# simonmeister/UnFlow

Hardware: AMD Instinct MI355X
Metric: image-pairs/s (fwd+bwd) FlowNetC 384x512 (higher is better)
Workload: dtype f32; 1 GPU; FlowNetC unsupervised step: bidirectional fwd + census/2nd-order loss pyramid + bwd + L2/Adam, 4 pairs/GPU, 384x512, 441-ch correlation (BASELINE configs[1]); global_batch=4, height=384, width=512, parallelism=dp1, hipgraph=True

## Files before the change

### include/unflow_hip.h

```cpp
#ifndef UNFLOW_HIP_H_
#define UNFLOW_HIP_H_

#include <stddef.h>

#ifdef __cplusplus
extern "C" {
#endif

typedef void* unflow_stream_t;
typedef struct unflow_planes unflow_planes;

#define UNFLOW_OK 0
#define UNFLOW_ERR_NULL (-1)
#define UNFLOW_ERR_EMPTY_OUTPUT (-2)
#define UNFLOW_ERR_EVEN_KERNEL (-3)
#define UNFLOW_ERR_NOT_DIVISIBLE (-4)
#define UNFLOW_ERR_SHAPE (-5)
#define UNFLOW_ERR_UNSUPPORTED (-7)
#define UNFLOW_ERR_LAUNCH (-8)
#define UNFLOW_ERR_WORKSPACE (-9)

const char* unflow_status_string(int status);
int unflow_version(void);

// ... 216 lines not shown

size_t unflow_conv_pl_workspace_bytes(int B, int H, int W, int Cin, int Cout, int k, int stride, int n_planes);

size_t unflow_flow_wgrad_batched_workspace_bytes(int n, const int* kind, const int* B, const int* H, const int* W, const int* Cin);
int unflow_flow_wgrad_batched(int n, const int* kind, const float* const* x, const int* ldx, const float* const* dz,
                              const int* lddz, float* const* dw, const int* B, const int* H, const int* W, const int* Cin,
                              void* workspace, size_t workspace_bytes, unflow_stream_t stream);

int unflow_debug_work_order(int mt, int nt, int ncls, int nsplit, int order, int xcd, int* out, int out_blocks);

int unflow_comm_available(void);
int unflow_comm_unique_id(void* id128);
int unflow_comm_init(const void* id128, int nranks, int rank, void** comm);
int unflow_comm_info(void* comm, int* nranks, int* rank);
int unflow_allreduce_sum_f32(float* buf, long n, void* comm, unflow_stream_t stream);
int unflow_comm_destroy(void* comm);

int unflow_debug_streamk_plan(int G, int mtp, int nt, int nchunk, int ncls, const int* ntaps, int ngroups, int* range_pos, int npos,
                              const int* pos, int* decoded);
int unflow_debug_streamk_timeouts(void);

int unflow_conv2d_fwd_pl(const float* x, int ldx, const unflow_planes* x_pl, const float* w, const unflow_planes* w_pl,
                         const float* bias, float* y, int ldy, const unflow_planes* y_pl, int B, int H, int W, int Cin,
                         int Cout, int k, int stride, int leaky, void* workspace, size_t workspace_bytes,
                         unflow_stream_t stream);
int unflow_conv2d_bwd_data_pl(const float* dz, int lddz, const unflow_planes* dz_pl, const float* w,
                              const unflow_planes* w_pl, float* dx, int lddx, const unflow_planes* dx_pl, int pl_lo,
                              int pl_hi, int B, int H, int W, int Cin, int Cout, int k, int stride, int accumulate,
                              const float* act_src, int ld_act, const unflow_planes* act_pl, int act_lo, int act_hi,
                              void* workspace, size_t workspace_bytes, unflow_stream_t stream);
int unflow_conv2d_bwd_filter_pl(const float* x, int ldx, const unflow_planes* x_pl, const float* dz, int lddz,
                                const unflow_planes* dz_pl, float* dw, int B, int H, int W, int Cin, int Cout, int k,
                                int stride, void* workspace, size_t workspace_bytes, unflow_stream_t stream);
int unflow_conv2d_transpose_fwd_pl(const float* x, int ldx, const unflow_planes* x_pl, const float* w,
                                   const unflow_planes* w_pl, const float* bias, float* y, int ldy,
                                   const unflow_planes* y_pl, int B, int H, int W, int Cin, int Cout, int leaky,
                                   void* workspace, size_t workspace_bytes, unflow_stream_t stream);
int unflow_conv2d_transpose_bwd_data_pl(const float* dz, int lddz, const unflow_planes* dz_pl, const float* w,
                                        const unflow_planes* w_pl, float* dx, int lddx, const unflow_planes* dx_pl,
                                        int pl_lo, int pl_hi, int B, int H, int W, int Cin, int Cout, int accumulate,
                                        const float* act_src, int ld_act, const unflow_planes* act_pl, int act_lo,
                                        int act_hi, void* workspace, size_t workspace_bytes, unflow_stream_t stream);
int unflow_conv2d_transpose_bwd_filter_pl(const float* x, int ldx, const unflow_planes* x_pl, const float* dz, int lddz,
                                          const unflow_planes* dz_pl, float* dw, int B, int H, int W, int Cin, int Cout,
                                          void* workspace, size_t workspace_bytes, unflow_stream_t stream);

int unflow_resize_bilinear_tf1(const float* in, float* out, int B, int H, int W, int C, int out_h, int out_w,
                               float scale, unflow_stream_t stream);

int unflow_supervised_flow_loss(const float* flow, int h, int w, const float* flow_gt, const float* mask_gt, float flow_scale,
                                float weight, float* loss_acc, float* d_flow, int accumulate, int B, int H, int W,
                                unflow_stream_t stream);

int unflow_stack_input_pair(const float* first4, const float* second4, const float* prev_flow2, float* out, int ld_out, int N,
                            int H, int W, int h, int w, float flow_scale, unflow_stream_t stream);
int unflow_stack_input_pair_bwd(const float* d_out, int ld_out, const float* first4, const float* second4,
                                const float* prev_flow2, float* d_prev_flow2, int N, int H, int W, int h, int w,
                                float flow_scale, unflow_stream_t stream);

int unflow_adam_step(float* p, const float* grad, float* m, float* v, long n, long n_regularized, float grad_scale,
                     float l2_scale, float lr_t, float beta1, float beta2, float eps, unflow_stream_t stream);

int unflow_adam_step_regloss(float* p, const float* grad, float* m, float* v, long n, long n_regularized,
                             float grad_scale, float l2_scale, float lr_t, float beta1, float beta2, float eps,
                             float* loss_acc, unflow_stream_t stream);

// ... 107 lines not shown
```

### unflow_amd/core/engine.py

```python
import math
import os
from collections import OrderedDict

import numpy as np
import torch

from .. import _lib
from .._lib import check, ptr, stream, cf, cl
from . import layers as L

FLOW_SCALE = 5.0
CHANNEL_MEAN = [104.920005, 110.1753, 114.785955]
LAYER_WEIGHTS = [12.7, 4.35, 3.9, 3.4, 1.1]
LAYER_PATCH_DISTANCES = [3, 2, 2, 1, 1]
LAYER_WEIGHTS_FULL_RES = [12.7, 5.5, 5.0, 4.35, 3.9, 3.4, 1.1]
LAYER_PATCH_DISTANCES_FULL_RES = [3, 3] + LAYER_PATCH_DISTANCES
L2_SCALE = 0.0004
LOSSES = ['occ', 'sym', 'fb', 'grad', 'ternary', 'photo', 'smooth_1st', 'smooth_2nd']

DEFAULT_PARAMS = dict(flownet='C', pyramid_loss=True, border_mask=True, ternary_weight=1.0, smooth_2nd_weight=3.0)


def pad4(c):
    return (c + 3) // 4 * 4


def round8(c):
    return (c + 7) // 8 * 8


def conv_math_mode():
    m = os.environ.get('UNFLOW_CONV_MATH', 'bf16x3')
    if m not in ('bf16x3', 'fp32', 'f16'):
        raise ValueError("UNFLOW_CONV_MATH must be bf16x3, fp32 or f16")
    return m


RGB4_FORM = True


class Layer:
    __slots__ = ('name', 'kind', 'k', 'cin', 'cout', 'stride', 'act', 'cin_p', 'cout_p', 'in_map', 'w', 'b', 'dw', 'db', 'mw', 'vw', 'mb', 'vb',
                 'wpl_d', 'wpl_t')

    def __init__(self, name, kind, k, cin, cout, stride, act, in_map=None, cin_p=None):
        self.name, self.kind, self.k, self.cin, self.cout, self.stride, self.act = name, kind, k, cin, cout, stride, act
        self.in_map = in_map or [(0, 0, cin)]
        if cin_p is None:
            cin_p = cin if (kind == 'deconv' and cin == 2) else pad4(max(lo + n for lo, _, n in self.in_map))
        self.cin_p = cin_p
        self.cout_p = cout if cout <= 2 else pad4(cout)
        self.wpl_d = self.wpl_t = None

    def wshape(self):
        if self.kind == 'conv':
            return (self.k, self.k, self.cin_p, self.cout_p)
        return (self.k, self.k, self.cout_p, self.cin_p)

    def tf_wshape(self):
        return (self.k, self.k, self.cin, self.cout) if self.kind == 'conv' else (self.k, self.k, self.cout, self.cin)

    def wplane_view(self):
        if self.kind == 'conv' and self.k == 7 and self.stride == 2 and self.cin_p == 4 and RGB4_FORM:
            return (7, 28, self.cout_p)
        return (self.k * self.k, self.wshape()[2], self.wshape()[3])

    def uses_planes(self):
        return self.cout > 4 and self.cin_p >= 4


def concat_layout(parts):
    off, d = 0, {}
    for nm, n in parts:
        off = pad4(off)
        d[nm] = (off, n)
        off += n
    return d, pad4(off)


class ActView(dict):

    def __init__(self, stage):
        super().__init__()
        self._stage = stage

# ... 393 lines not shown
            if e.wgrad_sync_each:
                main.wait_stream(side)

        flow_jobs = []
        n_flow = sum(1 for op, _, _, _ in self.bwd[lo:hi] if op.kind == 'layer' and op.l.cout <= 2) if e.batch_flow_wgrad else 0

        for k, (op, first, act_lo, act_hi) in enumerate(self.bwd[lo:hi], lo):
            if op.kind == 'corr':
                c3, g3, gout = self.pt(op.src), self.pt(op.src, True), self.pt(op.dst, True)
                C = op.src[2] - op.src[1]
                h8, w8 = e.H // 8, e.W // 8
                assert first
                pl = self._corr_planes(c3)
                if e.supervised:
                    p0, p1 = (None, None) if pl is None else (_lib.planes_of(pl[:, :B]), _lib.planes_of(pl[:, B:]))
                    check(_lib.lib().unflow_correlation_nhwc_bwd_pl(ptr(gout.t), gout.t.stride(2), ptr(c3.t[:B]), ptr(c3.t[B:]),
                                                                    c3.t.stride(2), p0, p1, 0, ptr(g3.t[:B]), ptr(g3.t[B:]),
                                                                    g3.t.stride(2), 0, B, C, h8, w8, 1, 20, 20, 1, 2, e.stream()),
                          "correlation_grad")
                else:
                    c3pl = _lib.planes_of(pl)
                    check(_lib.lib().unflow_correlation_nhwc_bwd_pl(ptr(gout.t), gout.t.stride(2), ptr(c3.t), ptr(c3.t),
                                                                    c3.t.stride(2), c3pl, c3pl, B, ptr(g3.t), ptr(None),
                                                                    g3.t.stride(2), 1, N, C, h8, w8, 1, 20, 20, 1, 2, e.stream()),
                          "correlation_grad")
                for r0, r1, clo, chi in self.bwd_post_act.get(k, ()):
                    self._leaky_bwd_rows(g3, c3, r0, r1, clo, chi)
                continue
            l = op.l
            x, dz = _rows(self.pt(op.src), op.n), _rows(self.pt(op.dst, True), op.n)
            if l.cout_p != l.cout:
                dz = L.PT(dz.t.as_strided(dz.t.shape[:3] + (l.cout_p,), dz.t.stride(), dz.t.storage_offset()), dz.pl, dz.scale)
            if e._bias_plan is None:
                e._bias_jobs.append((dz.t, l))
            xv = op.src[0] not in self.planes_only
            wg = (L.conv_bwd_filter, (x, dz, l.dw, l.stride, xv)) if l.kind == 'conv' else (L.deconv_bwd_filter, (x, dz, l.dw, xv))
            if n_flow and l.cout <= 2:
                flow_jobs.append((l.kind, x, dz, l.dw))
                wg = (L.flow_wgrad_batched, (flow_jobs,)) if len(flow_jobs) == n_flow else None
            if wg is None:
                pass
            elif side is None or (e.wgrad_inline_tiny and l.cout <= 2):
                wg[0](*wg[1])
            else:
                pending.append(wg)
                if len(pending) >= e.wgrad_group:
                    flush()
            sb = op.src[0]
            is_input = sb == 'x0' or (sb == self.bin and op.src[1] == 0 and op.src[2] == pad4(self.in_ch)
                                      and op.l.name.endswith('conv1'))
            if sb not in self.Gd or (is_input and not self.need_in_grad):
                continue
            dx = _rows(self.pt(op.src, True), op.n)
            accumulate = (not first) or sb.startswith('flow')
            if k in self.bwd_zero_rows:
                r0, r1 = self.bwd_zero_rows[k]
                gz = self.Gd[sb].t[r0:r1]
                check(_lib.lib().unflow_zero(ptr(gz), _lib.csz(gz.numel() * 4), e.stream()), "zero")
            act_src = _rows(self.pt(op.src), op.n) if act_hi > act_lo else None
            apl = sb in self.planes_only
            if l.kind == 'conv':
                L.conv_bwd_data(dz, l.w, l.wpl_d, dx, l.stride, accumulate, act_src, act_lo, act_hi, act_planes=apl)
            else:
                L.deconv_bwd_data(dz, l.w, l.wpl_t, dx, accumulate, act_src, act_lo, act_hi, act_planes=apl)
        if side is not None:
            flush()
        if before_join is not None:
            before_join()
        if side is not None:
# ... 996 lines not shown
```

### unflow_amd/core/layers.py

```python
import torch

from .. import _lib
from .._lib import check, ptr, stream, csz
from ..ops import workspace


def nhwc(t):
    assert t.dim() == 4 and t.dtype == torch.float32 and t.is_cuda, "NHWC float32 CUDA tensor expected"
    B, H, W, C = t.shape
    ld = t.stride(2)
    assert t.stride(3) == 1 and t.stride(1) == W * ld and t.stride(0) == H * W * ld, \
        "tensor must be a channel-slice view of a contiguous NHWC buffer"
    return ptr(t), ld, B, H, W, C


def out_hw(H, W, stride):
    return -(-H // stride), -(-W // stride)


_WS_SLOT = [1]


class ws_slot:

# ... 155 lines not shown
    k = w.shape[0]
    assert tuple(w.shape) == (k, k, Cin, Cout) and w.is_contiguous() and (Ho, Wo) == out_hw(H, W, stride)
    wsp, wsn = _ws_pl(x.t.device, B, H, W, Cin, Cout, k, stride, _npl(x, y))
    check(_lib.lib().unflow_conv2d_fwd_pl(xp, ldx, x.planes(), ptr(w), _lib.planes_of(w_pl), ptr(bias), yp, ldy,
                                          y.planes(), B, H, W, Cin, Cout, k, stride, int(bool(leaky)), wsp, wsn,
                                          stream()), "conv2d_fwd_pl")


def _act_args(act_src, act_planes):
    if act_src is None:
        return ptr(None), 0, None
    a = _pt(act_src)
    if act_planes:
        assert a.pl is not None
        return ptr(None), 0, a.planes()
    ap, lda = nhwc(a.t)[:2]
    return ap, lda, None


def conv_bwd_data(dz, w, w_pl, dx, stride, accumulate=False, act_src=None, act_lo=0, act_hi=0, act_planes=False):
    dz, dx = _pt(dz), _pt(dx)
    dzp, lddz, B, Ho, Wo, Cout = nhwc(dz.t)
    dxp, lddx, _, H, W, Cin = nhwc(dx.t)
    k = w.shape[0]
    assert tuple(w.shape) == (k, k, Cin, Cout)
    ap, lda, apl = _act_args(act_src, act_planes)
    wsp, wsn = _ws_pl(dz.t.device, B, H, W, Cin, Cout, k, stride, _npl(dz, dx))
    check(_lib.lib().unflow_conv2d_bwd_data_pl(dzp, lddz, dz.planes(), ptr(w), _lib.planes_of(w_pl), dxp, lddx,
                                               dx.planes(), act_lo, act_hi, B, H, W, Cin, Cout, k, stride,
                                               int(bool(accumulate)), ap, lda, apl, act_lo, act_hi, wsp, wsn, stream()),
          "conv2d_bwd_data_pl")


def conv_bwd_filter(x, dz, dw, stride, x_fp32=True):
    x, dz = _pt(x), _pt(dz)
    xp, ldx, B, H, W, Cin = nhwc(x.t)
    if not x_fp32:
        assert x.pl is not None
        xp = ptr(None)
    dzp, lddz, _, Ho, Wo, Cout = nhwc(dz.t)
    k = dw.shape[0]
    assert tuple(dw.shape) == (k, k, Cin, Cout) and dw.is_contiguous()
    wsp, wsn = _ws_pl(x.t.device, B, H, W, Cin, Cout, k, stride, _npl(x, dz))
    check(_lib.lib().unflow_conv2d_bwd_filter_pl(xp, ldx, x.planes(), dzp, lddz, dz.planes(), ptr(dw), B, H,
                                                 W, Cin, Cout, k, stride, wsp, wsn, stream()), "conv2d_bwd_filter_pl")


def deconv_fwd(x, w, w_pl, bias, y, leaky, planes_only=False):
    x, y = _pt(x), _pt(y)
    xp, ldx, B, H, W, Cin = nhwc(x.t)
    yp, ldy, _, Ho, Wo, Cout = nhwc(y.t)
    if planes_only:
        assert y.pl is not None
        yp = ptr(None)
    assert tuple(w.shape) == (4, 4, Cout, Cin) and (Ho, Wo) == (2 * H, 2 * W)
    wsp, wsn = _ws_pl(x.t.device, B, 2 * H, 2 * W, Cin, Cout, 4, 2, _npl(x, y))
    check(_lib.lib().unflow_conv2d_transpose_fwd_pl(xp, ldx, x.planes(), ptr(w), _lib.planes_of(w_pl), ptr(bias), yp,
                                                    ldy, y.planes(), B, H, W, Cin, Cout, int(bool(leaky)), wsp, wsn,
                                                    stream()), "conv2d_transpose_fwd_pl")


def deconv_bwd_data(dz, w, w_pl, dx, accumulate=False, act_src=None, act_lo=0, act_hi=0, act_planes=False):
    dz, dx = _pt(dz), _pt(dx)
    dzp, lddz, B, Ho, Wo, Cout = nhwc(dz.t)
    dxp, lddx, _, H, W, Cin = nhwc(dx.t)
    assert tuple(w.shape) == (4, 4, Cout, Cin) and (Ho, Wo) == (2 * H, 2 * W)
    ap, lda, apl = _act_args(act_src, act_planes)
    wsp, wsn = _ws_pl(dz.t.device, B, Ho, Wo, Cin, Cout, 4, 2, _npl(dz, dx))
    check(_lib.lib().unflow_conv2d_transpose_bwd_data_pl(dzp, lddz, dz.planes(), ptr(w), _lib.planes_of(w_pl), dxp,
                                                         lddx, dx.planes(), act_lo, act_hi, B, H, W, Cin, Cout,
                                                         int(bool(accumulate)), ap, lda, apl, act_lo, act_hi, wsp, wsn,
                                                         stream()),
          "conv2d_transpose_bwd_data_pl")


def deconv_bwd_filter(x, dz, dw, x_fp32=True):
# ... 47 lines not shown
```

### unflow_amd/csrc/conv_planes.hip

```cpp
#include "igemm_shared.h"
#include "planes_shared.h"
#include "halo_kernel.h"

namespace {
using namespace igemm;

template <int BM, int BN, int WM, int WN, int NPL, bool F16>
__global__ __launch_bounds__(256, (NPL == 3 && BM == 128 && BN == 128) ? 3 : 1) void igemm_pl_gather_kernel(const PlGatherParams p) {
  constexpr int TM = WM / 32, TN = WN / 32;
  constexpr int WAVES_N = BN / WN;
  static_assert((BM / WM) * WAVES_N == 4, "4 waves");
  static_assert(BM % 64 == 0 && BN % 64 == 0, "row passes of 64");
  constexpr int A_PLANE = BM * LDH, B_PLANE = BN * LDH;
  constexpr int AR = BM / 64, NB = BN / 64;
  constexpr int NT = NPL == 3 ? 6 : 1;

  extern __shared__ __attribute__((aligned(16))) unsigned short smem16[];
  const int tid = threadIdx.x, lane = tid & 63, wid = tid >> 6;
  unsigned short* Ah = smem16;
  unsigned short* Bh = Ah + NPL * A_PLANE;
  int* pix = reinterpret_cast<int*>(reinterpret_cast<char*>(smem16) + pl_gather_main_bytes(BM, BN, WN, NPL));

  const int wm = wid / WAVES_N, wn = wid % WAVES_N;
  int mtile, ntile, cls_id, split;
// ... 1766 lines not shown
UNFLOW_API int unflow_adam_planes_batched(int n, float* const* w, const int* taps, const int* R, const int* Cc, void* const* direct,
                                          void* const* transposed, const int* regularized, int n_planes, float* P, const float* G,
                                          float* M, float* V, float grad_scale, float l2_scale, float lr_t, float beta1, float beta2,
                                          float eps, float* loss_acc, unflow_stream_t stream) {
  if (!w || !taps || !R || !Cc || !direct || !transposed || !regularized || !P || !G || !M || !V) return UNFLOW_ERR_NULL;
  if (n_planes != 0 && n_planes != 1 && n_planes != 3) return UNFLOW_ERR_UNSUPPORTED;
  hipStream_t st = as_stream(stream);
  AdamPlaneArgs a{P, G, M, V, grad_scale, l2_scale, lr_t, beta1, beta2, eps, loss_acc};
  for (int i0 = 0; i0 < n; i0 += MAX_WDESC) {
    WPlaneBatch b{};
    b.n = min(n - i0, MAX_WDESC);
    b.n_planes = n_planes ? n_planes : 3;
    unsigned long long reg_mask = 0;
    int blocks = 0;
    for (int i = 0; i < b.n; i++) {
      WPlaneDesc& d = b.d[i];
      if (!w[i0 + i] || taps[i0 + i] <= 0 || R[i0 + i] <= 0 || Cc[i0 + i] <= 0 || w[i0 + i] < P) return UNFLOW_ERR_SHAPE;
      if (!n_planes && (direct[i0 + i] || transposed[i0 + i])) return UNFLOW_ERR_UNSUPPORTED;
      d.w = w[i0 + i];
      d.direct = reinterpret_cast<unsigned short*>(direct[i0 + i]);
      d.transposed = reinterpret_cast<unsigned short*>(transposed[i0 + i]);
      d.taps = taps[i0 + i]; d.R = R[i0 + i]; d.Cc = Cc[i0 + i];
      d.tiles_r = cdiv(d.R, 64);
      d.tiles_c = cdiv(d.Cc, 64);
      d.block0 = blocks;
      blocks += d.taps * d.tiles_r * d.tiles_c;
      if (regularized[i0 + i]) reg_mask |= 1ull << i;
    }
    if (blocks > 0) adam_planes_kernel<<<blocks, 256, 0, st>>>(b, a, reg_mask);
  }
  return launch_status();
}

static int pl_gather_nsplit(const GatherGeom& g, int npl) {
  int bn;
  if (!pl_halo_ok(g)) return plan_pl_gather(g, npl).nsplit;
  return plan_pl_halo(g, npl, &bn);
}

UNFLOW_API size_t unflow_conv_pl_workspace_bytes(int B, int H, int W, int Cin, int Cout, int k, int stride, int n_planes) {
  if (B <= 0 || H <= 0 || W <= 0 || Cin <= 0 || Cout <= 0 || k <= 0 || stride <= 0) return 0;
  size_t need = unflow_conv_workspace_bytes(B, H, W, (Cin + 3) & ~3, Cout, k, stride);
  if (Cout <= 4 || (n_planes != 1 && n_planes != 3)) return need;
  const int Ci8 = (Cin + 7) & ~7, Co8 = (Cout + 7) & ~7;
  GatherGeom g{};
  build_conv_fwd(g, B, H, W, Ci8, Cout, k, stride);
  need = max(need, pl_gather_partial_bytes(g, pl_gather_nsplit(g, n_planes)));
  if (unflow::options().streamk > 0 && n_planes == 3) need = max(need, pl_halo_sk_ws_bytes());
  if (stride == 2 && build_conv_fwd_s2acc(g, B, H, W, Ci8, Cout, k) && pl_halo_acc_pays(g))
    need = max(need, pl_gather_partial_bytes(g, pl_gather_nsplit(g, n_planes)));
  GatherGeom d{};
  if ((stride == 1 || stride == 2) && build_conv_dgrad(d, B, H, W, Cin, Co8, k, stride) == UNFLOW_OK)
    need = max(need, pl_gather_partial_bytes(d, pl_gather_nsplit(d, n_planes)));
  WgradGeom wg{};
  build_conv_wgrad(wg, B, H, W, Ci8, Cout, k, stride);
  need = max(need, pl_wgrad_plan_bytes(wg, Cin, n_planes));
  if (Cin == 4 && k == 7 && stride == 2 && W % 2 == 0) {
    g.Cs = 32; g.KW = 1; g.wtaps = 7; g.cls[0].ntx = 1;
    need = max(need, pl_gather_partial_bytes(g, pl_gather_nsplit(g, n_planes)));
    wg.Ca = 32; wg.KW = 1;
    need = max(need, pl_wgrad_plan_bytes(wg, 28, n_planes));
  }
  if (k == 4 && stride == 2 && H % 2 == 0 && W % 2 == 0) {
    GatherGeom tf{};
    build_deconv_fwd(tf, B, H / 2, W / 2, Ci8, Cout);
    need = max(need, pl_gather_partial_bytes(tf, pl_gather_nsplit(tf, n_planes)));
    GatherGeom td{};
    build_deconv_dgrad(td, B, H / 2, W / 2, Cin, Co8);
    need = max(need, pl_gather_partial_bytes(td, pl_gather_nsplit(td, n_planes)));
    build_deconv_dgrad_acc(td, B, H / 2, W / 2, Cin, Co8);
    if (pl_halo_acc_pays(td)) need = max(need, pl_gather_partial_bytes(td, pl_gather_nsplit(td, n_planes)));
    WgradGeom tw{};
    build_deconv_wgrad(tw, B, H / 2, W / 2, Cin, Co8);
    need = max(need, pl_wgrad_plan_bytes(tw, Cout, n_planes));
  }
  return need + 1024;
}

int conv_first7_fwd(const unflow_planes* x_pl, const unflow_planes* w_pl, const float* bias, const unflow_planes* y_pl, int B, int H,
                    int W, int Cout, int leaky, hipStream_t st);

static bool rgb4_form(const unflow_planes* x_pl, int W, int Cin, int k, int stride) {
  return x_pl && x_pl->base && Cin == 4 && k == 7 && stride == 2 && x_pl->ld == 4 && W % 2 == 0 &&
         (x_pl->n_planes == 1 || x_pl->n_planes == 3) && (reinterpret_cast<uintptr_t>(x_pl->base) & 7) == 0;
}

static bool use_planes(const unflow_planes* a, int ca, const unflow_planes* b, int cb, int Cout_or_n) {
  return Cout_or_n > 4 && planes_ok(a, ca) && planes_ok(b, cb) && a->n_planes == b->n_planes;
}

UNFLOW_API int unflow_conv2d_fwd_pl(const float* x, int ldx, const unflow_planes* x_pl, const float* w,
                                    const unflow_planes* w_pl, const float* bias, float* y, int ldy,
                                    const unflow_planes* y_pl, int B, int H, int W, int Cin, int Cout, int k, int stride,
                                    int leaky, void* workspace, size_t workspace_bytes, unflow_stream_t stream) {
// ... 25 lines not shown
  p.src_inv = 1.f / (plane_scale(x_pl) * plane_scale(w_pl));
  p.bias = bias; p.dst = y; p.ldd = ldy; p.act_src = nullptr; p.leaky = leaky; p.accumulate = 0;
  p.pl = plane_out(y_pl, 0, Cout);
  return run_pl_gather(p, x_pl->n_planes, workspace, workspace_bytes, as_stream(stream));
}

UNFLOW_API int unflow_conv2d_bwd_data_pl(const float* dz, int lddz, const unflow_planes* dz_pl, const float* w,
                                         const unflow_planes* w_pl, float* dx, int lddx, const unflow_planes* dx_pl,
                                         int pl_lo, int pl_hi, int B, int H, int W, int Cin, int Cout, int k, int stride,
                                         int accumulate, const float* act_src, int ld_act, const unflow_planes* act_pl,
                                         int act_lo, int act_hi, void* workspace, size_t workspace_bytes,
                                         unflow_stream_t stream) {
  if ((!dx && !(dx_pl && dx_pl->base)) || (!dz && !dz_pl)) return UNFLOW_ERR_NULL;
  if (B <= 0 || H <= 0 || W <= 0 || Cin <= 0 || Cout <= 0 || k <= 0 || (stride != 1 && stride != 2)) return UNFLOW_ERR_SHAPE;
  const int Co8 = (Cout + 7) & ~7;
  const bool pointwise32 = k == 1 && stride == 1 && Cout == 32;
  if (pointwise32 || !use_planes(dz_pl, Cout, w_pl, Cout, Cout) || w_pl->ld != Co8)
    return (!dx || (!act_src && act_pl && act_hi > act_lo)) ? UNFLOW_ERR_UNSUPPORTED : unflow_conv2d_bwd_data_po(dz, lddz, w, dx, lddx, B, H, W, Cin, Cout, k, stride, accumulate, act_src, ld_act, act_lo,
                                     act_hi, plane_out(dx_pl, pl_lo, pl_hi), workspace, workspace_bytes, stream);
  if (dx && lddx < Cin) return UNFLOW_ERR_UNSUPPORTED;
  PlGatherParams p{};
  const int bc = build_conv_dgrad(p, B, H, W, Cin, Co8, k, stride);
  if (bc != UNFLOW_OK) return bc;
  p.src = reinterpret_cast<const unsigned short*>(dz_pl->base); p.src_ps = dz_pl->plane_stride; p.lds = dz_pl->ld;
  p.w = reinterpret_cast<const unsigned short*>(w_pl->base); p.w_ps = w_pl->plane_stride;
  p.src_inv = 1.f / (plane_scale(dz_pl) * plane_scale(w_pl));
  p.bias = nullptr; p.dst = dx; p.ldd = lddx; p.act_lo = act_lo; p.act_hi = act_hi;
  set_act(p, act_src, ld_act, act_pl);
  p.leaky = 0; p.accumulate = accumulate;
  p.pl = plane_out(dx_pl, pl_lo, pl_hi);
  return run_pl_gather(p, dz_pl->n_planes, workspace, workspace_bytes, as_stream(stream));
}

UNFLOW_API int unflow_conv2d_bwd_filter_pl(const float* x, int ldx, const unflow_planes* x_pl, const float* dz, int lddz,
                                           const unflow_planes* dz_pl, float* dw, int B, int H, int W, int Cin, int Cout,
                                           int k, int stride, void* workspace, size_t workspace_bytes,
                                           unflow_stream_t stream) {
  if (!dw || (!x && !x_pl) || (!dz && !dz_pl)) return UNFLOW_ERR_NULL;
  if (B <= 0 || H <= 0 || W <= 0 || Cin <= 0 || Cout <= 0 || k <= 0 || stride <= 0) return UNFLOW_ERR_SHAPE;
  const bool rgb4 = rgb4_form(x_pl, W, Cin, k, stride) && planes_ok(dz_pl, Cout) && dz_pl->n_planes == x_pl->n_planes &&
                    Cout > 4 && Cout % 4 == 0;
  if (!rgb4 && (!use_planes(x_pl, Cin, dz_pl, Cout, Cout) || Cout % 4 != 0))
    return (!x || !dz) ? UNFLOW_ERR_UNSUPPORTED :
           unflow_conv2d_bwd_filter(x, ldx, dz, lddz, dw, nullptr, B, H, W, Cin, Cout, k, stride, workspace, workspace_bytes, stream);
  PlWgradParams p{};
  build_conv_wgrad(p, B, H, W, (Cin + 7) & ~7, Cout, k, stride);
  if (rgb4) { p.Ca = 32; p.KW = 1; p.gpx = 2; }
  p.src = reinterpret_cast<const unsigned short*>(x_pl->base); p.src_ps = x_pl->plane_stride; p.lds = x_pl->ld;
  p.dst = reinterpret_cast<const unsigned short*>(dz_pl->base); p.dst_ps = dz_pl->plane_stride; p.ldd = dz_pl->ld;
  p.out_scale = 1.f / (plane_scale(x_pl) * plane_scale(dz_pl));
  p.out = dw; p.Ca_out = rgb4 ? 28 : Cin;
  size_t used = 0;
  return run_pl_wgrad(p, x_pl->n_planes, workspace, workspace_bytes, &used, as_stream(stream));
}

UNFLOW_API int unflow_conv2d_transpose_fwd_pl(const float* x, int ldx, const unflow_planes* x_pl, const float* w,
                                              const unflow_planes* w_pl, const float* bias, float* y, int ldy,
                                              const unflow_planes* y_pl, int B, int H, int W, int Cin, int Cout, int leaky,
                                              void* workspace, size_t workspace_bytes, unflow_stream_t stream) {
  if ((!y && !(y_pl && y_pl->base)) || (!x && !x_pl)) return UNFLOW_ERR_NULL;
  if (B <= 0 || H <= 0 || W <= 0 || Cin <= 0 || Cout <= 0) return UNFLOW_ERR_SHAPE;
  const int Ci8 = (Cin + 7) & ~7;
  if (!use_planes(x_pl, Cin, w_pl, Cin, Cout) || w_pl->ld != Ci8)
    return !y ? UNFLOW_ERR_UNSUPPORTED : unflow_conv2d_transpose_fwd_po(x, ldx, w, bias, y, ldy, B, H, W, Cin, Cout, leaky, plane_out(y_pl, 0, Cout), workspace,
                                          workspace_bytes, stream);
  if (y && ldy < Cout) return UNFLOW_ERR_UNSUPPORTED;
  PlGatherParams p{};
  build_deconv_fwd(p, B, H, W, Ci8, Cout);
  p.src = reinterpret_cast<const unsigned short*>(x_pl->base); p.src_ps = x_pl->plane_stride; p.lds = x_pl->ld;
  p.w = reinterpret_cast<const unsigned short*>(w_pl->base); p.w_ps = w_pl->plane_stride;
  p.src_inv = 1.f / (plane_scale(x_pl) * plane_scale(w_pl));
  p.bias = bias; p.dst = y; p.ldd = ldy; p.act_src = nullptr; p.leaky = leaky; p.accumulate = 0;
  p.pl = plane_out(y_pl, 0, Cout);
  return run_pl_gather(p, x_pl->n_planes, workspace, workspace_bytes, as_stream(stream));
}

UNFLOW_API int unflow_conv2d_transpose_bwd_data_pl(const float* dz, int lddz, const unflow_planes* dz_pl, const float* w,
                                                   const unflow_planes* w_pl, float* dx, int lddx,
                                                   const unflow_planes* dx_pl, int pl_lo, int pl_hi, int B, int H, int W,
                                                   int Cin, int Cout, int accumulate, const float* act_src, int ld_act,
                                                   const unflow_planes* act_pl, int act_lo, int act_hi, void* workspace,
                                                   size_t workspace_bytes, unflow_stream_t stream) {
  if ((!dx && !(dx_pl && dx_pl->base)) || (!dz && !dz_pl)) return UNFLOW_ERR_NULL;
  if (B <= 0 || H <= 0 || W <= 0 || Cin <= 0 || Cout <= 0) return UNFLOW_ERR_SHAPE;
  const int Co8 = (Cout + 7) & ~7;
  if (!use_planes(dz_pl, Cout, w_pl, Cout, Cout) || w_pl->ld != Co8 || Cin <= 4)
// ... 39 lines not shown
```

### unflow_amd/csrc/options.h

```cpp
#pragma once

#define UNFLOW_OPTION_LIST(X)                                                                                              \
  X(conv_math_fp32, 0)           \
  X(wgrad_math_fp32, 0)                             \
  X(corr_math_fp32, 0)                                                               \
  X(gather_min_kt, 8)                          \
  X(gather_max_split, 16)                                                           \
  X(wgrad_min_kt, 8)                     \
  X(gather_pp, 1)          \
  X(gather_pp_fill, 60)    \
  X(f16_k64, 1)            \
  X(f16_wgrad_dma, 1)      \
  X(f16_tall, 0)           \
  X(f16_db, 0)             \
  X(gather_tile2d, 1)                                                     \
  X(conv1_direct, 1)       \
  X(halo, 1)                                     \
  X(streamk, 1)                \
  X(streamk_groups, 8)             \
  X(halo_max_split, 16)                                         \
  X(halo_s2, 1)                       \
  X(xcd_swizzle, 1)                                                                        \
  X(wgrad_dma, 1)                                                \
  X(wgrad_pp, 1)                                                     \
  X(corr_nb, 1)                                                               \
  X(corr_rs, 2)            \
  X(corr_wb, 1)                                                                 \
  X(corr_rw, 1)                                                       \
  X(corr_bwd_b128, 1)                                                 \
  X(corr_bwd_rot, -1)              \
  X(corr_bwd_planes, 1)                                                 \
  X(corr_bwd_share, 1)

namespace unflow {
struct Options {
#define X(name, def) int name = def;
  UNFLOW_OPTION_LIST(X)
#undef X
};
Options& options();
}
```

Measured before the change: 688.6 image-pairs/s.

## Add dedicated first-layer 7x7 wgrad kernel with fused bias gradient

Adds a specialized MFMA kernel for the weight gradient of the first 7x7 stride-2 conv on RGB4 planes. It uses LDS transpose reads and a software-pipelined tile loop with per-block partial slabs, then a tree reduction. A ones-row trick folds the bias gradient into the same GEMM, so that layer's separate bias-reduction job is dropped. It is enabled by default behind a new option, and adds workspace and extra code paths with their own shape and alignment checks.

New measurement: 690.9 image-pairs/s (median of 2 runs). About the same (+0.3%).

```diff
diff --git a/include/unflow_hip.h b/include/unflow_hip.h
--- a/include/unflow_hip.h
+++ b/include/unflow_hip.h
@@ -272,6 +272,11 @@
 int unflow_conv2d_bwd_filter_pl(const float* x, int ldx, const unflow_planes* x_pl, const float* dz, int lddz,
                                 const unflow_planes* dz_pl, float* dw, int B, int H, int W, int Cin, int Cout, int k,
                                 int stride, void* workspace, size_t workspace_bytes, unflow_stream_t stream);
+int unflow_conv2d_bwd_filter_bias_pl(const float* x, int ldx, const unflow_planes* x_pl, const float* dz, int lddz,
+                                     const unflow_planes* dz_pl, float* dw, float* db, int B, int H, int W, int Cin, int Cout,
+                                     int k, int stride, void* workspace, size_t workspace_bytes, unflow_stream_t stream);
+int unflow_conv2d_bwd_filter_bias_pl_supported(const unflow_planes* x_pl, const unflow_planes* dz_pl, int B, int H, int W,
+                                               int Cin, int Cout, int k, int stride, size_t workspace_bytes);
 int unflow_conv2d_transpose_fwd_pl(const float* x, int ldx, const unflow_planes* x_pl, const float* w,
                                    const unflow_planes* w_pl, const float* bias, float* y, int ldy,
                                    const unflow_planes* y_pl, int B, int H, int W, int Cin, int Cout, int leaky,
diff --git a/unflow_amd/core/engine.py b/unflow_amd/core/engine.py
--- a/unflow_amd/core/engine.py
+++ b/unflow_amd/core/engine.py
@@ -41,7 +41,7 @@
 
 class Layer:
     __slots__ = ('name', 'kind', 'k', 'cin', 'cout', 'stride', 'act', 'cin_p', 'cout_p', 'in_map', 'w', 'b', 'dw', 'db', 'mw', 'vw', 'mb', 'vb',
-                 'wpl_d', 'wpl_t')
+                 'wpl_d', 'wpl_t', 'db_fused')
 
     def __init__(self, name, kind, k, cin, cout, stride, act, in_map=None, cin_p=None):
         self.name, self.kind, self.k, self.cin, self.cout, self.stride, self.act = name, kind, k, cin, cout, stride, act
@@ -51,6 +51,7 @@
         self.cin_p = cin_p
         self.cout_p = cout if cout <= 2 else pad4(cout)
         self.wpl_d = self.wpl_t = None
+        self.db_fused = False
 
     def wshape(self):
         if self.kind == 'conv':
@@ -510,9 +511,12 @@
             if l.cout_p != l.cout:
                 dz = L.PT(dz.t.as_strided(dz.t.shape[:3] + (l.cout_p,), dz.t.stride(), dz.t.storage_offset()), dz.pl, dz.scale)
             if e._bias_plan is None:
-                e._bias_jobs.append((dz.t, l))
+                l.db_fused = l.kind == 'conv' and l.cout_p == l.cout and L.conv_bwd_filter_bias_ok(x, dz, l.dw, l.stride)
+                if not l.db_fused:
+                    e._bias_jobs.append((dz.t, l))
             xv = op.src[0] not in self.planes_only
-            wg = (L.conv_bwd_filter, (x, dz, l.dw, l.stride, xv)) if l.kind == 'conv' else (L.deconv_bwd_filter, (x, dz, l.dw, xv))
+            wg = (L.conv_bwd_filter, (x, dz, l.dw, l.stride, xv, l.db if l.db_fused else None)) if l.kind == 'conv' \
+                else (L.deconv_bwd_filter, (x, dz, l.dw, xv))
             if n_flow and l.cout <= 2:
                 flow_jobs.append((l.kind, x, dz, l.dw))
                 wg = (L.flow_wgrad_batched, (flow_jobs,)) if len(flow_jobs) == n_flow else None
diff --git a/unflow_amd/core/layers.py b/unflow_amd/core/layers.py
--- a/unflow_amd/core/layers.py
+++ b/unflow_amd/core/layers.py
@@ -211,7 +211,18 @@
           "conv2d_bwd_data_pl")
 
 
-def conv_bwd_filter(x, dz, dw, stride, x_fp32=True):
+def conv_bwd_filter_bias_ok(x, dz, dw, stride):
+    x, dz = _pt(x), _pt(dz)
+    if x.pl is None or dz.pl is None:
+        return False
+    _, _, B, H, W, Cin = nhwc(x.t)
+    Cout = dz.t.shape[-1]
+    k = dw.shape[0]
+    _, wsn = _ws_pl(x.t.device, B, H, W, Cin, Cout, k, stride, _npl(x, dz))
+    return bool(_lib.lib().unflow_conv2d_bwd_filter_bias_pl_supported(x.planes(), dz.planes(), B, H, W, Cin, Cout, k, stride, wsn))
+
+
+def conv_bwd_filter(x, dz, dw, stride, x_fp32=True, db=None):
     x, dz = _pt(x), _pt(dz)
     xp, ldx, B, H, W, Cin = nhwc(x.t)
     if not x_fp32:
@@ -221,6 +232,12 @@
     k = dw.shape[0]
     assert tuple(dw.shape) == (k, k, Cin, Cout) and dw.is_contiguous()
     wsp, wsn = _ws_pl(x.t.device, B, H, W, Cin, Cout, k, stride, _npl(x, dz))
+    if db is not None:
+        assert db.numel() == Cout and db.is_contiguous()
+        check(_lib.lib().unflow_conv2d_bwd_filter_bias_pl(xp, ldx, x.planes(), dzp, lddz, dz.planes(), ptr(dw), ptr(db), B, H,
+                                                          W, Cin, Cout, k, stride, wsp, wsn, stream()),
+              "conv2d_bwd_filter_bias_pl")
+        return
     check(_lib.lib().unflow_conv2d_bwd_filter_pl(xp, ldx, x.planes(), dzp, lddz, dz.planes(), ptr(dw), B, H,
                                                  W, Cin, Cout, k, stride, wsp, wsn, stream()), "conv2d_bwd_filter_pl")
 
diff --git a/unflow_amd/csrc/conv_first_wgrad.hip b/unflow_amd/csrc/conv_first_wgrad.hip
--- /dev/null
+++ b/unflow_amd/csrc/conv_first_wgrad.hip
@@ -0,0 +1,284 @@
+#include "planes_shared.h"
+
+namespace {
+using namespace igemm;
+
+struct First7WgradParams {
+  const unsigned short* x;
+  long x_ps;
+  const unsigned short* dz;
+  long dz_ps;
+  int ldd;
+  float* partial;
+  int B, H, W, Ho, Wo;
+  int pieces, ntiles, per;
+};
+
+constexpr int G_SLAB = 7 * 32 * 64;
+
+template <int NS, int TS>
+struct G {
+  static constexpr int KS = TS / 16;
+  static constexpr int XG = TS + 3;
+  static constexpr int XPITCH = (XG + 1) * 16;
+  static constexpr int XPLANE = 7 * XPITCH;
+  static constexpr int DPLANE = TS * 128;
+  static constexpr int SMEM = 3 * XPLANE + 3 * DPLANE;
+  static constexpr int THREADS = 448 * NS;
+  static constexpr int NX = (3 * 7 * XG + THREADS - 1) / THREADS;
+  static constexpr int ND = (3 * TS * 8 + THREADS - 1) / THREADS;
+  static constexpr int NTW = 2 / NS;
+};
+
+__device__ __forceinline__ int dz_swz(int k, int g) {
+  const int sw = ((k >> 1) & 1) << 1;
+  return k * 64 + ((((g >> 1) ^ sw) << 1) | (g & 1)) * 8;
+}
+
+__device__ __forceinline__ s16x8 ld_tr8(const unsigned char* p, int second) {
+  const s16x4 lo = __builtin_amdgcn_ds_read_tr16_b64_v4i16((s16x4 __attribute__((address_space(3)))*)(p));
+  const s16x4 hi = __builtin_amdgcn_ds_read_tr16_b64_v4i16((s16x4 __attribute__((address_space(3)))*)(p + second));
+  return __builtin_shufflevector(lo, hi, 0, 1, 2, 3, 4, 5, 6, 7);
+}
+
+template <int NS, int TS, int MINW, bool PIPE>
+__global__ __launch_bounds__(448 * NS, MINW) void conv_first7_wgrad_kernel(const First7WgradParams p) {
+  using C = G<NS, TS>;
+  constexpr int NX = C::NX, ND = C::ND, NTW = C::NTW, THREADS = C::THREADS;
+  extern __shared__ __attribute__((aligned(16))) unsigned char gsm[];
+  unsigned char* Xl = gsm;
+  unsigned char* Dl = gsm + 3 * C::XPLANE;
+  const int tid = threadIdx.x, lane = tid & 63;
+  const int wid = __builtin_amdgcn_readfirstlane(tid >> 6);
+  const int ky = wid / NS;
+  const int nt0 = (wid % NS) * NTW;
+
+  const int x_pb = (int)(p.x_ps * 2), dz_pb = (int)(p.dz_ps * 2);
+  const int ldd2 = p.ldd * 2;
+  const __amdgpu_buffer_rsrc_t x_rs = make_rsrc(p.x, (size_t)2 * x_pb + (size_t)p.B * p.H * p.W * 8);
+  const __amdgpu_buffer_rsrc_t dz_rs = make_rsrc(p.dz, (size_t)2 * dz_pb + (((size_t)p.B * p.Ho * p.Wo - 1) * (size_t)p.ldd + 64) * 2);
+
+  int x_src[NX], x_row[NX], x_px[NX], x_lds[NX];
+#pragma unroll
+  for (int i = 0; i < NX; i++) {
+    const int idx = tid + i * THREADS;
+    const bool any = idx < 3 * 7 * C::XG;
+    const int pl = idx / (7 * C::XG), rem = idx - pl * (7 * C::XG);
+    const int r = rem / C::XG, g = rem - r * C::XG;
+    x_src[i] = pl * x_pb + (r * p.W + 2 * g) * 8;
+    x_row[i] = r;
+    x_px[i] = 2 * g;
+    x_lds[i] = any ? pl * C::XPLANE + r * C::XPITCH + g * 16 : -1;
+  }
+  int d_src[ND], d_site[ND], d_lds[ND];
+#pragma unroll
+  for (int i = 0; i < ND; i++) {
+    const int idx = tid + i * THREADS;
+    const bool any = idx < 3 * TS * 8;
+    const int pl = idx / (TS * 8), rem = idx - pl * (TS * 8);
+    const int s = rem >> 3, g = rem & 7;
+    d_src[i] = pl * dz_pb + s * ldd2 + g * 16;
+    d_site[i] = s;
+    d_lds[i] = any ? pl * C::DPLANE + dz_swz(s, g) * 2 : -1;
+  }
+  u32x4 xl[NX], dl[ND];
+  auto tile_of = [&](int t, int& b, int& oy, int& ox0) {
+    oy = t % p.Ho;
+    t /= p.Ho;
+    const int pc = t % p.pieces;
+    b = t / p.pieces;
+    ox0 = pc * TS;
+  };
+  const int t0 = blockIdx.x * p.per, t1 = min(p.ntiles, t0 + p.per);
+  auto load_tile = [&](int t) {
+    int b, oy, ox0;
+    tile_of(t, b, oy, ox0);
+    const bool live = t < t1;
+    const unsigned hlim = live ? (unsigned)p.H : 0u, wlim = live ? (unsigned)p.W : 0u;
+    const int wolim = live ? p.Wo : 0;
+    const int y0 = 2 * oy - 2, px0 = 2 * ox0 - 2;
+    const int xbase = ((b * p.H + y0) * p.W + px0) * 8, dbase = ((b * p.Ho + oy) * p.Wo + ox0) * ldd2;
+#pragma unroll
+    for (int i = 0; i < NX; i++) {
+      const int ok = ((unsigned)(y0 + x_row[i]) < hlim) & ((unsigned)(px0 + x_px[i]) < wlim) & (x_lds[i] >= 0);
+      xl[i] = buf_ld16(x_rs, ok ? x_src[i] + xbase : OOB_MARK);
+    }
+#pragma unroll
+    for (int i = 0; i < ND; i++) {
+      const int ok = (ox0 + d_site[i] < wolim) & (d_lds[i] >= 0);
+      dl[i] = buf_ld16(dz_rs, ok ? d_src[i] + dbase : OOB_MARK);
+    }
+  };
+
+  const int i16 = lane & 15, grp16 = lane >> 4, lh = grp16 >> 1, l31 = lane & 31;
+  const int krow = 8 * lh + (i16 >> 2);
+  const int c = 16 * (grp16 & 1) + 4 * (i16 & 3);
+  const unsigned char* a_rd = Xl + ky * C::XPITCH + krow * 16 + c * 2;
+  const unsigned char* b_rd[NTW];
+#pragma unroll
+  for (int j = 0; j < NTW; j++) b_rd[j] = Dl + (dz_swz(krow, (c + 32 * (nt0 + j)) >> 3) + (c & 7)) * 2;
+  const bool ones_row = ky == 0 && l31 == 28;
+  s16x8 one8, zero8;
+#pragma unroll
+  for (int e = 0; e < 8; e++) { one8[e] = (short)0x3F80; zero8[e] = 0; }
+
+  f32x16 acc[NTW];
+#pragma unroll
+  for (int j = 0; j < NTW; j++)
+#pragma unroll
+    for (int e = 0; e < 16; e++) acc[j][e] = 0.f;
+
+  auto rd = [&](int ks, s16x8 (&a)[3], s16x8 (&b)[NTW][3]) __attribute__((always_inline)) {
+#pragma unroll
+    for (int pl = 0; pl < 3; pl++) {
+      a[pl] = ld_tr8(a_rd + pl * C::XPLANE + ks * 256, 64);
+#pragma unroll
+      for (int j = 0; j < NTW; j++) b[j][pl] = ld_tr8(b_rd[j] + pl * C::DPLANE + ks * 2048, 512);
+    }
+  };
+
+  if (t0 < t1) load_tile(t0);
+#pragma unroll 1
+  for (int t = t0; t < t1; t++) {
+    __syncthreads();
+#pragma unroll
+    for (int i = 0; i < NX; i++)
+      if (x_lds[i] >= 0) *reinterpret_cast<u32x4*>(Xl + x_lds[i]) = xl[i];
+#pragma unroll
+    for (int i = 0; i < ND; i++)
+      if (d_lds[i] >= 0) *reinterpret_cast<u32x4*>(Dl + d_lds[i]) = dl[i];
+    __syncthreads();
+    load_tile(t + 1);
+    s16x8 af[2][3], bf[2][NTW][3];
+    rd(0, af[0], bf[0]);
+    if (PIPE) __builtin_amdgcn_sched_barrier(0);
+#pragma unroll
+    for (int ks = 0; ks < C::KS; ks++) {
+      const int cur = ks & 1;
+      if (ks + 1 < C::KS) rd(ks + 1, af[cur ^ 1], bf[cur ^ 1]);
+      const s16x8 a[3] = {ones_row ? one8 : af[cur][0], ones_row ? zero8 : af[cur][1], ones_row ? zero8 : af[cur][2]};
+#pragma unroll
+      for (int tt = 0; tt < 6; tt++)
+#pragma unroll
+        for (int j = 0; j < NTW; j++) mfma_terms<3, false>(a, bf[cur][j], acc[j], tt);
+      if (PIPE && ks + 1 < C::KS) {
+#pragma unroll
+        for (int i = 0; i < 6; i++) {
+          __builtin_amdgcn_sched_group_barrier(0x008, 1, 0);
+          __builtin_amdgcn_sched_group_barrier(0x100, 1 + NTW, 0);
+        }
+        __builtin_amdgcn_sched_group_barrier(0x008, 6 * NTW - 6, 0);
+      }
+      if (PIPE) __builtin_amdgcn_sched_barrier(0);
+    }
+  }
+
+  float* o = p.partial + (size_t)blockIdx.x * G_SLAB + ky * (32 * 64);
+#pragma unroll
+  for (int r = 0; r < 16; r++) {
+    const int m = (r & 3) + 8 * (r >> 2) + 4 * (lane >> 5);
+#pragma unroll
+    for (int j = 0; j < NTW; j++) o[m * 64 + 32 * (nt0 + j) + l31] = acc[j][r];
+  }
+}
+
+__global__ void first7_wgrad_finish_kernel(const float* __restrict__ partial, int S, float* __restrict__ dw, float* __restrict__ db) {
+  const int e = blockIdx.x * blockDim.x + threadIdx.x;
+  if (e >= G_SLAB) return;
+  const int n = e & 63, m = (e >> 6) & 31, ky = e >> 11;
+  if (m > 28 || (m == 28 && (ky != 0 || !db))) return;
+  float v = 0.f;
+  int s = 0;
+  for (; s + 8 <= S; s += 8) {
+    float q[8];
+#pragma unroll
+    for (int k = 0; k < 8; k++) q[k] = partial[(size_t)(s + k) * G_SLAB + e];
+#pragma unroll
+    for (int k = 0; k < 8; k++) v += q[k];
+  }
+  for (; s < S; s++) v += partial[(size_t)s * G_SLAB + e];
+  if (m < 28) dw[(ky * 28 + m) * 64 + n] = v;
+  else db[n] = v;
+}
+
+int first7_wgrad_cus() {
+  static int cus = 0;
+  if (!cus) {
+    int dev = 0;
+    hipDeviceProp_t prop;
+    if (hipGetDevice(&dev) == hipSuccess && hipGetDeviceProperties(&prop, dev) == hipSuccess) cus = prop.multiProcessorCount;
+    if (cus <= 0) cus = 256;
+  }
+  return cus;
+}
+
+constexpr int G_NS = 1, G_TS = 128;
+
+int first7_wgrad_grid(int B, int H, int W, int* per_out) {
+  const int Ho = H / 2, Wo = W / 2;
+  const int ntiles = B * Ho * cdiv(Wo, G_TS);
+  const int per = cdiv(ntiles, first7_wgrad_cus());
+  if (per_out) *per_out = per;
+  return cdiv(ntiles, per);
+}
+
+template <int NS, int TS, int MINW, bool PIPE>
+void launch_first7_wgrad(const First7WgradParams& p, int grid, hipStream_t st) {
+  static DynLdsBook attr_book{};
+  (void)ensure_dyn_lds(reinterpret_cast<const void*>(&conv_first7_wgrad_kernel<NS, TS, MINW, PIPE>), G<NS, TS>::SMEM, attr_book);
+  conv_first7_wgrad_kernel<NS, TS, MINW, PIPE><<<grid, G<NS, TS>::THREADS, G<NS, TS>::SMEM, st>>>(p);
+}
+
+}
+
+size_t conv_first7_wgrad_ws_bytes(int B, int H, int W) {
+  if (B <= 0 || H < 2 || W < 2) return 0;
+  const int S = first7_wgrad_grid(B, H, W, nullptr);
+  return (size_t)S * G_SLAB * sizeof(float) + reduce_scratch_bytes(G_SLAB, S);
+}
+
+int conv_first7_wgrad_ok(const unflow_planes* x_pl, const unflow_planes* dz_pl, int B, int H, int W, int Cout, size_t ws_bytes) {
+  if (!unflow::options().conv1_wgrad_direct) return UNFLOW_ERR_UNSUPPORTED;
+  if (Cout != 64 || !x_pl || !dz_pl || !x_pl->base || !dz_pl->base || x_pl->n_planes != 3 || dz_pl->n_planes != 3)
+    return UNFLOW_ERR_UNSUPPORTED;
+  if (x_pl->ld != 4 || dz_pl->ld < 64 || dz_pl->ld % 8 != 0 || H % 2 != 0 || W % 2 != 0 || B <= 0 || H < 2 || W < 2)
+    return UNFLOW_ERR_UNSUPPORTED;
+  if ((reinterpret_cast<uintptr_t>(x_pl->base) & 15) || (x_pl->plane_stride & 7) || (reinterpret_cast<uintptr_t>(dz_pl->base) & 15) ||
+      (dz_pl->plane_stride & 7))
+    return UNFLOW_ERR_UNSUPPORTED;
+  const float sx = x_pl->scale, sd = dz_pl->scale;
+  if ((sx != 0.f && sx != 1.f) || (sd != 0.f && sd != 1.f)) return UNFLOW_ERR_UNSUPPORTED;
+  const int Ho = H / 2, Wo = W / 2;
+  if (x_pl->plane_stride < 0 || dz_pl->plane_stride < 0 || (size_t)4 * x_pl->plane_stride + (size_t)B * H * W * 8 > 0x3fffffffu ||
+      (size_t)4 * dz_pl->plane_stride + ((size_t)B * Ho * Wo * dz_pl->ld) * 2 > 0x3fffffffu)
+    return UNFLOW_ERR_UNSUPPORTED;
+  if (ws_bytes < conv_first7_wgrad_ws_bytes(B, H, W)) return UNFLOW_ERR_UNSUPPORTED;
+  return UNFLOW_OK;
+}
+
+int conv_first7_wgrad(const unflow_planes* x_pl, const unflow_planes* dz_pl, float* dw, float* db, int B, int H, int W, int Cout,
+                      void* ws, size_t ws_bytes, hipStream_t st) {
+  const int ok = conv_first7_wgrad_ok(x_pl, dz_pl, B, H, W, Cout, ws ? ws_bytes : 0);
+  if (ok != UNFLOW_OK) return ok;
+  if ((reinterpret_cast<uintptr_t>(ws) & 15) != 0) return UNFLOW_ERR_UNSUPPORTED;
+  First7WgradParams p{};
+  p.x = reinterpret_cast<const unsigned short*>(x_pl->base); p.x_ps = x_pl->plane_stride;
+  p.dz = reinterpret_cast<const unsigned short*>(dz_pl->base); p.dz_ps = dz_pl->plane_stride; p.ldd = dz_pl->ld;
+  p.B = B; p.H = H; p.W = W; p.Ho = H / 2; p.Wo = W / 2;
+  p.pieces = cdiv(p.Wo, G_TS);
+  p.ntiles = B * p.Ho * p.pieces;
+  int S = first7_wgrad_grid(B, H, W, &p.per);
+  p.partial = reinterpret_cast<float*>(ws);
+  launch_first7_wgrad<G_NS, G_TS, 2, true>(p, S, st);
+  const float* partial = p.partial;
+  float* scratch = p.partial + (size_t)S * G_SLAB;
+  while (S > REDUCE_FAN) {
+    const int G = (S + REDUCE_FAN - 1) / REDUCE_FAN;
+    launch_sum_partials(partial, scratch, G_SLAB, S, G, st);
+    partial = scratch;
+    scratch = scratch + (size_t)G * G_SLAB;
+    S = G;
+  }
+  first7_wgrad_finish_kernel<<<cdiv(G_SLAB, 256), 256, 0, st>>>(partial, S, dw, db);
+  return launch_status();
+}
diff --git a/unflow_amd/csrc/conv_planes.hip b/unflow_amd/csrc/conv_planes.hip
--- a/unflow_amd/csrc/conv_planes.hip
+++ b/unflow_amd/csrc/conv_planes.hip
@@ -1822,6 +1822,11 @@
   return launch_status();
 }
 
+size_t conv_first7_wgrad_ws_bytes(int B, int H, int W);
+int conv_first7_wgrad_ok(const unflow_planes* x_pl, const unflow_planes* dz_pl, int B, int H, int W, int Cout, size_t ws_bytes);
+int conv_first7_wgrad(const unflow_planes* x_pl, const unflow_planes* dz_pl, float* dw, float* db, int B, int H, int W, int Cout,
+                      void* ws, size_t ws_bytes, hipStream_t st);
+
 static int pl_gather_nsplit(const GatherGeom& g, int npl) {
   int bn;
   if (!pl_halo_ok(g)) return plan_pl_gather(g, npl).nsplit;
@@ -1850,6 +1855,7 @@
     need = max(need, pl_gather_partial_bytes(g, pl_gather_nsplit(g, n_planes)));
     wg.Ca = 32; wg.KW = 1;
     need = max(need, pl_wgrad_plan_bytes(wg, 28, n_planes));
+    if (Cout == 64 && n_planes == 3 && H % 2 == 0) need = max(need, conv_first7_wgrad_ws_bytes(B, H, W));
   }
   if (k == 4 && stride == 2 && H % 2 == 0 && W % 2 == 0) {
     GatherGeom tf{};
@@ -1941,14 +1947,18 @@
   return run_pl_gather(p, dz_pl->n_planes, workspace, workspace_bytes, as_stream(stream));
 }
 
-UNFLOW_API int unflow_conv2d_bwd_filter_pl(const float* x, int ldx, const unflow_planes* x_pl, const float* dz, int lddz,
-                                           const unflow_planes* dz_pl, float* dw, int B, int H, int W, int Cin, int Cout,
-                                           int k, int stride, void* workspace, size_t workspace_bytes,
-                                           unflow_stream_t stream) {
+static int conv2d_bwd_filter_pl(const float* x, int ldx, const unflow_planes* x_pl, const float* dz, int lddz,
+                                const unflow_planes* dz_pl, float* dw, float* db, int B, int H, int W, int Cin, int Cout, int k,
+                                int stride, void* workspace, size_t workspace_bytes, unflow_stream_t stream) {
   if (!dw || (!x && !x_pl) || (!dz && !dz_pl)) return UNFLOW_ERR_NULL;
   if (B <= 0 || H <= 0 || W <= 0 || Cin <= 0 || Cout <= 0 || k <= 0 || stride <= 0) return UNFLOW_ERR_SHAPE;
   const bool rgb4 = rgb4_form(x_pl, W, Cin, k, stride) && planes_ok(dz_pl, Cout) && dz_pl->n_planes == x_pl->n_planes &&
                     Cout > 4 && Cout % 4 == 0;
+  if (rgb4) {
+    const int code = conv_first7_wgrad(x_pl, dz_pl, dw, db, B, H, W, Cout, workspace, workspace_bytes, as_stream(stream));
+    if (code != UNFLOW_ERR_UNSUPPORTED) return code;
+  }
+  if (db) return UNFLOW_ERR_UNSUPPORTED;
   if (!rgb4 && (!use_planes(x_pl, Cin, dz_pl, Cout, Cout) || Cout % 4 != 0))
     return (!x || !dz) ? UNFLOW_ERR_UNSUPPORTED :
            unflow_conv2d_bwd_filter(x, ldx, dz, lddz, dw, nullptr, B, H, W, Cin, Cout, k, stride, workspace, workspace_bytes, stream);
@@ -1961,6 +1971,26 @@
   p.out = dw; p.Ca_out = rgb4 ? 28 : Cin;
   size_t used = 0;
   return run_pl_wgrad(p, x_pl->n_planes, workspace, workspace_bytes, &used, as_stream(stream));
+}
+
+UNFLOW_API int unflow_conv2d_bwd_filter_pl(const float* x, int ldx, const unflow_planes* x_pl, const float* dz, int lddz,
+                                           const unflow_planes* dz_pl, float* dw, int B, int H, int W, int Cin, int Cout,
+                                           int k, int stride, void* workspace, size_t workspace_bytes,
+                                           unflow_stream_t stream) {
+  return conv2d_bwd_filter_pl(x, ldx, x_pl, dz, lddz, dz_pl, dw, nullptr, B, H, W, Cin, Cout, k, stride, workspace, workspace_bytes, stream);
+}
+
+UNFLOW_API int unflow_conv2d_bwd_filter_bias_pl(const float* x, int ldx, const unflow_planes* x_pl, const float* dz, int lddz,
+                                                const unflow_planes* dz_pl, float* dw, float* db, int B, int H, int W, int Cin,
+                                                int Cout, int k, int stride, void* workspace, size_t workspace_bytes,
+                                                unflow_stream_t stream) {
+  return conv2d_bwd_filter_pl(x, ldx, x_pl, dz, lddz, dz_pl, dw, db, B, H, W, Cin, Cout, k, stride, workspace, workspace_bytes, stream);
+}
+
+UNFLOW_API int unflow_conv2d_bwd_filter_bias_pl_supported(const unflow_planes* x_pl, const unflow_planes* dz_pl, int B, int H, int W,
+                                                          int Cin, int Cout, int k, int stride, size_t workspace_bytes) {
+  if (B <= 0 || H <= 0 || W <= 0 || !rgb4_form(x_pl, W, Cin, k, stride) || !planes_ok(dz_pl, Cout)) return 0;
+  return conv_first7_wgrad_ok(x_pl, dz_pl, B, H, W, Cout, workspace_bytes) == UNFLOW_OK ? 1 : 0;
 }
 
 UNFLOW_API int unflow_conv2d_transpose_fwd_pl(const float* x, int ldx, const unflow_planes* x_pl, const float* w,
diff --git a/unflow_amd/csrc/options.h b/unflow_amd/csrc/options.h
--- a/unflow_amd/csrc/options.h
+++ b/unflow_amd/csrc/options.h
@@ -15,6 +15,7 @@
   X(f16_db, 0)             \
   X(gather_tile2d, 1)                                                     \
   X(conv1_direct, 1)       \
+  X(conv1_wgrad_direct, 1)  \
   X(halo, 1)                                     \
   X(streamk, 1)                \
   X(streamk_groups, 8)             \
```
